# evandez/neuron-descriptions

Hardware: AMD Instinct MI355X
Metric: neuron-descriptions/sec (whole node), 4096 neurons x k=15 exemplars (higher is better)
Workload: dtype f32-equivalent: operands split into (hi,lo) f16 pairs (22 significant bits), 3 f16 MFMAs per product, f32 accumulate

## Files before the change

### neuron-descriptions_amd/csrc/chain.hip

```cpp
#include "common.h"

#include <cstdlib>

namespace milan {

typedef float f32x16 __attribute__((ext_vector_type(16)));
typedef float f32x4 __attribute__((ext_vector_type(4)));
typedef _Float16 f16x8 __attribute__((ext_vector_type(8)));

#define GLOBAL_AS __attribute__((address_space(1)))
#define LDS_AS __attribute__((address_space(3)))

namespace {

__device__ inline f16x8 h8(f32x4 v) { return __builtin_bit_cast(f16x8, v); }

__device__ inline void chain_split8(const float* v, f32x4* hi_out, f32x4* lo_out) {
  split8_rne(v, hi_out, lo_out);
}
__device__ inline void chain_join8(f32x4 hi, f32x4 lo, float* v) { join8_exact(hi, lo, v); }

constexpr int kSRow = 68;
constexpr int kTileFloats = 64 * 64;
constexpr int kConvMaxW = 56;
// ... 5 lines not shown
}

}

template <int P, int NW, bool RES_LDS, int KD, bool XACC, bool PROF = false, int NR = P,
          bool CONV = false, bool C1 = false>
__global__ __launch_bounds__(NW * 64, NW / 4) void chain_kernel(ChainArgs g) {
  long long tprof[8] = {0, 0, 0, 0, 0, 0, 0, 0};
  long long tlast = 0;
  auto stamp = [&](int k) {
    if constexpr (PROF) {
      const long long t = __builtin_readcyclecounter();
      tprof[k] += t - tlast;
      tlast = t;
    }
  };
  if constexpr (PROF) tlast = __builtin_readcyclecounter();
  constexpr int N3 = 4 * P, N1 = NR;
  constexpr int K3 = P + KD;
  constexpr int KS3 = K3 / 16;
  constexpr int NSLAB = N3 / 64;
  constexpr int T3 = K3 / 64;
  constexpr bool RES = KD == 0;
  static_assert(!(RES_LDS && !RES) && K3 % 64 == 0, "chain: configuration");
  constexpr int T1 = N1 / 64;
  constexpr int L = T3 + T1;
  constexpr int NT1 = N1 / 32;
  constexpr int STAGES = RES_LDS ? 7 : 4, AHEAD = STAGES - 1;
  constexpr int INFL = AHEAD - 2;
  constexpr int PIECES = 16 / NW;
  constexpr int C_OPS = RES_LDS ? 8 : (RES ? 10 : 2);
  static_assert(P % 64 == 0 && (NW == 4 || NW == 8), "chain: configuration");
  static_assert(!CONV || (P == 64 && NW == 8 && !RES_LDS), "chain: the conv front needs planes 64");
  static_assert(!C1 || CONV, "chain: c1 in front needs the conv front");
  constexpr int Q1 = C1 ? 1 : 0;
  constexpr int QC = CONV ? 9 + Q1 : 0;
  extern __shared__ __attribute__((aligned(16))) float smem[];

  const int tid = threadIdx.x;
  const int lane = tid & 63;
  const int wave = __builtin_amdgcn_readfirstlane(tid >> 6);
  const int px = lane & 31, half = lane >> 5;
  float sat = 0.f;
  float* ring = smem;
  float* strip = smem + STAGES * kTileFloats + wave * (32 * kSRow);
  float* rstrip = strip;
  float* biasl = smem + STAGES * kTileFloats + NW * (32 * kSRow);

  g.M = live_rows(g.m_live, g.m_live_mul, g.M);
  if ((long)blockIdx.x * (NW * 32) >= g.M) return;
  const long m0 = (long)blockIdx.x * (NW * 32) + wave * 32;
  const long mfrag = (m0 + px < g.M) ? m0 + px : (long)g.M - 1;
  const bool tail = (long)(blockIdx.x + 1) * (NW * 32) > g.M;

  const int lrow = lane >> 4;
  const int lpos = lane & 15;
  auto issue_tile = [&](int q) {
    constexpr int NTILES = QC + NSLAB * L;
    q = q < NTILES ? q : NTILES - 1;
    const float* base;
    long ld;
    if (C1 && q == 0) {
      base = g.W0; ld = 64;
    } else if (CONV && q < QC) {
      base = g.W2 + 64 * (q - Q1); ld = 9 * 64;
    } else {
      const int qc = q - QC;
      const int j = qc / L, qq = qc - j * L;
      if (qq < T3) { base = g.W3 + (long)(64 * j) * K3 + 64 * qq; ld = K3; }
      else { base = g.W1 + (long)(64 * (qq - T3)) * N3 + 64 * j; ld = N3; }
    }
    float* slot = ring + (q % STAGES) * kTileFloats;
#pragma unroll
    for (int i = 0; i < PIECES; ++i) {
      const int pc = wave * PIECES + i;
      const int rr = 4 * pc + lrow;
      const int c = lpos ^ (rr & 15);
      __builtin_amdgcn_global_load_lds(
          (const GLOBAL_AS void*)(base + (long)rr * ld + c * 4),
          (LDS_AS void*)(slot + pc * 256), 16, 0, 0);
    }
  };

  f32x4 t2h[KS3], t2l[KS3];
  float* const cin = smem + STAGES * kTileFloats;
  float* const czero = cin + kConvSlots * 64;
  f32x4 bias2v[CONV ? 8 : 1], bias0v[C1 ? 8 : 1];
  if constexpr (C1) {
#pragma unroll
    for (int s4 = 0; s4 < 4; ++s4) {
      bias0v[2 * s4] = *reinterpret_cast<const f32x4*>(g.bias0 + 16 * s4 + 8 * half);
      bias0v[2 * s4 + 1] = *reinterpret_cast<const f32x4*>(g.bias0 + 16 * s4 + 8 * half + 4);
    }
  }
  if constexpr (CONV) {
    const long wg0 = (long)blockIdx.x * (NW * 32);
    const int nslots = NW * 32 + 2 * (g.cw + 1);
    const int npieces = (nslots + 3) >> 2;
    for (int pc = wave; pc < npieces; pc += NW) {
      const int sl = 4 * pc + lrow;
      long m = wg0 - (g.cw + 1) + sl;
      m = m < 0 ? 0 : (m < g.M ? m : (long)g.M - 1);
      const int c = lpos ^ (sl & 15);
      __builtin_amdgcn_global_load_lds((const GLOBAL_AS void*)(g.C2in + m * 64 + c * 4),
                                       (LDS_AS void*)(cin + pc * 256), 16, 0, 0);
    }
// ... 314 lines not shown
        }

      }
      stamp(2);
      if (qq == T3 - 1) {
        const int n = 64 * j + ecol;
        f32x4 bias0, bias1, rh4[4], rl4[4];
        if constexpr (RES_LDS) {
          wait_vmcnt<(L * PIECES < 63 ? L * PIECES : 63)>();
          bias0 = *reinterpret_cast<const f32x4*>(biasl + n);
          bias1 = *reinterpret_cast<const f32x4*>(biasl + n + 4);
#pragma unroll
          for (int it = 0; it < 4; ++it) {
            const int row = it * 8 + erow;
            const float* rp = rstrip + row * 64;
            const int rsw = row & 1;
            rh4[it] = *reinterpret_cast<const f32x4*>(rp + (((ecol >> 2)) ^ rsw) * 4);
            rl4[it] = *reinterpret_cast<const f32x4*>(rp + (((ecol >> 2) + 1) ^ rsw) * 4);
          }
        } else {
          bias0 = bias3v[0]; bias1 = bias3v[1];
        }
#pragma unroll
        for (int t = 0; t < 2; ++t) {
          acc3[t] = acc3[t] * g.scale3;
          to_strip(acc3[t], t);
        }
#pragma unroll
        for (int it = 0; it < 4; ++it) {
          const int row = it * 8 + erow;
          const long m = m0 + row;
          float* sp = strip + row * kSRow + ecol;
          const f32x4 v0 = *reinterpret_cast<const f32x4*>(sp);
          const f32x4 v1 = *reinterpret_cast<const f32x4*>(sp + 4);
          f32x4 rh, rl;
          if constexpr (RES_LDS) {
            rh = rh4[it]; rl = rl4[it];
          } else if constexpr (RES) {
            rh = res[it][0]; rl = res[it][1];
          }
          float v[8], a[8];
#pragma unroll
          for (int e = 0; e < 4; ++e) {
            v[e] = v0[e] + bias0[e];
            v[4 + e] = v1[e] + bias1[e];
          }
          if constexpr (RES) {
            chain_join8(rh, rl, a);
#pragma unroll
            for (int e = 0; e < 8; ++e) v[e] = v[e] + a[e];
          }
          f32x4 hi, lo;
          split8_relu_rne(v, &hi, &lo, &sat);
          if (m < g.M) {
            float* xp = g.X + m * N3 + n;
            *reinterpret_cast<f32x4*>(xp) = hi;
            *reinterpret_cast<f32x4*>(xp + 4) = lo;
          }
          *reinterpret_cast<f32x4*>(sp) = hi;
          *reinterpret_cast<f32x4*>(sp + 4) = lo;
        }
        if constexpr (!RES_LDS) load_res(j + 1 < NSLAB ? j + 1 : j);
#pragma unroll
        for (int s = 0; s < 4; ++s) {
          const float* fp = strip + px * kSRow + (2 * s + half) * 8;
          xh[s] = *reinterpret_cast<const f32x4*>(fp);
          xl[s] = *reinterpret_cast<const f32x4*>(fp + 4);
        }
        if constexpr (RES_LDS) {
          asm volatile("s_waitcnt lgkmcnt(0)"
                       : "+v"(xh[0]), "+v"(xh[1]), "+v"(xh[2]), "+v"(xh[3]),
                         "+v"(xl[0]), "+v"(xl[1]), "+v"(xl[2]), "+v"(xl[3])
                       :: "memory");
          load_res(j + 1 < NSLAB ? j + 1 : j);
        }
      }
      stamp(3);
      {
        constexpr auto has_c = [](int i) { return ((i % L) + L) % L == T3 - 1; };
        int c_later = 0, c_first = 0;
#pragma unroll
        for (int d = 0; d <= INFL; ++d) {
          c_later += has_c(qq - d) ? 1 : 0;
          c_first += (qq - d >= 0 && has_c(qq - d)) ? 1 : 0;
        }
        const int cnt = (j == 0) ? c_first : c_later;
        constexpr int B = INFL * PIECES;
        if (tail) {
          wait_vmcnt<0>();
        } else {
          switch (cnt) {
            case 0: wait_vmcnt<B>(); break;
            case 1: wait_vmcnt<(B + C_OPS < 63 ? B + C_OPS : 63)>(); break;
            case 2: wait_vmcnt<(B + 2 * C_OPS < 63 ? B + 2 * C_OPS : 63)>(); break;
            default: wait_vmcnt<(B + 3 * C_OPS < 63 ? B + 3 * C_OPS : 63)>(); break;
          }
        }
      }
      stamp(4);
      __builtin_amdgcn_s_barrier();
      stamp(5);
    }
  }
  wait_vmcnt<0>();
  __builtin_amdgcn_s_barrier();

#pragma unroll
// ... 43 lines not shown
}

bool chain_conv_c1_supported(int P, int KD, int NR, int h, int w) {
  return chain_conv_supported(P, KD, NR, h, w) && KD == 64 && NR == 64;
}

bool chain_supported(int P, int KD, int NR) {
  if (NR == 2 * P) return KD == 0 && P == 64;
  if (NR != P) return false;
  if (KD == 0) return P == 64 || P == 128 || P == 256;
  return P == 64 && KD == 64;
}

template <int P, int NW, bool RES_LDS, int KD, bool XACC, bool PROF = false, int NR = P,
          bool CONV = false, bool C1 = false>
static int launch_chain_cfg(const ChainArgs& a, hipStream_t s) {
  size_t lds = sizeof(float) * (size_t)((RES_LDS ? 7 : 4) * kTileFloats +
                                        NW * 32 * kSRow + (RES_LDS ? 4 * P : 0));
  if (CONV) {
    const size_t with_region = sizeof(float) * (size_t)(4 * kTileFloats + kConvSlots * 64 + 64);
    lds = lds > with_region ? lds : with_region;
  }
  auto kern = chain_kernel<P, NW, RES_LDS, KD, XACC, PROF, NR, CONV, C1>;
  MILAN_TRY(ensure_lds_attr(reinterpret_cast<const void*>(kern), (int)lds));
  const int rows = NW * 32;
  const int grid = (a.M + rows - 1) / rows;
  hipLaunchKernelGGL(kern, dim3(grid), dim3(NW * 64), lds, s, a);
  MILAN_CHECK_HIP(hipGetLastError());
  return 0;
}

int launch_chain3(const ChainArgs& a, hipStream_t s);

int launch_chain(const ChainArgs& a0, hipStream_t s) {
  ChainArgs a = a0;
  if (a.status == nullptr) a.status = status_word();
  const int NR = a.NR ? a.NR : a.P;
  MILAN_REQUIRE(chain_supported(a.P, a.KD, NR) && a.M > 0, MILAN_ERR_SHAPE,
                "chain: unsupported planes %d (+%d) -> %d", a.P, a.KD, NR);
  auto al = [](const void* p) { return (reinterpret_cast<uintptr_t>(p) & 15) == 0; };
  const bool conv = a.C2in != nullptr;
  MILAN_REQUIRE(!conv || (chain_conv_supported(a.P, a.KD, NR, a.ch, a.cw) && a.W2 && a.bias2 &&
                          al(a.C2in) && al(a.W2) && al(a.bias2) && a.C2in != a.T1 &&
                          a.M % (a.ch * a.cw) == 0),
                MILAN_ERR_SHAPE, "chain: unsupported 3x3 front (%d x %d images)", a.ch, a.cw);
  const bool c1 = conv && a.W0 != nullptr;
  MILAN_REQUIRE(!c1 || (chain_conv_c1_supported(a.P, a.KD, NR, a.ch, a.cw) && a.bias0 && al(a.W0) &&
                        al(a.bias0)),
                MILAN_ERR_SHAPE, "chain: unsupported c1 front");
  MILAN_REQUIRE((conv || al(a.T2)) && al(a.W3) && al(a.bias3) && al(a.X) && al(a.W1) &&
                    al(a.bias1) && al(a.T1) &&
                    (a.KD ? (a.A2 && al(a.A2) && !a.R) : (a.R && al(a.R))),
                MILAN_ERR_SHAPE, "chain: operands must be 16-byte aligned");
  const double M = a.M, P = a.P, K3 = a.P + a.KD, R1 = NR;
  void* rec = gemm_profile_begin(
      2.0 * M * (4 * P) * (K3 + R1) + (conv ? 2.0 * M * 64 * 576 : 0.0) + (c1 ? 2.0 * M * 64 * 64 : 0.0),
      4.0 * (M * K3 + M * 4 * P * (a.KD ? 1 : 2) + M * R1 + 4 * P * (K3 + R1) +
             (conv ? 64.0 * 576 : 0.0)), s);
  profile_tag_kernel(a.P == 256 ? MILAN_KERNEL_CHAIN_WIDE
                                : (conv ? MILAN_KERNEL_BNECK : MILAN_KERNEL_CHAIN));
  int r;
#if MILAN_EXPERIMENTS
  if (conv && a.KD == 0 && NR == 64 && a.prof)
    r = launch_chain_cfg<64, 8, false, 0, true, true, 64, true>(a, s);
  else
#endif
  if (conv && NR == 128) r = launch_chain_cfg<64, 8, false, 0, false, false, 128, true>(a, s);
  else if (conv && a.KD == 0) r = launch_chain_cfg<64, 8, false, 0, true, false, 64, true>(a, s);
  else if (c1) r = launch_chain_cfg<64, 8, false, 64, true, false, 64, true, true>(a, s);
  else if (conv) r = launch_chain_cfg<64, 8, false, 64, true, false, 64, true>(a, s);
  else if (a.P == 256) r = launch_chain3(a, s);
  else if (a.P == 128) r = launch_chain_cfg<128, 8, false, 0, false>(a, s);
  else if (NR == 128) r = launch_chain_cfg<64, 8, false, 0, false, false, 128>(a, s);
  else if (a.KD == 0) r = launch_chain_cfg<64, 8, false, 0, true>(a, s);
  else r = launch_chain_cfg<64, 8, false, 64, true>(a, s);
  gemm_profile_end(rec, s);
  return r;
}

}
```

### neuron-descriptions_amd/csrc/common.h

```cpp
#pragma once
#include <hip/hip_runtime.h>
#include <stdint.h>
#include <stddef.h>
#include <string>
#include <vector>
#include <map>

#include "../../include/milan_hip.h"

#ifndef MILAN_EXPERIMENTS
#define MILAN_EXPERIMENTS 0
#endif

namespace milan {

void set_error(const char* fmt, ...);
#define MILAN_CHECK_HIP(expr)                                              \
  do {                                                                     \
    hipError_t _e = (expr);                                                \
    if (_e != hipSuccess) {                                                \
      milan::set_error("%s:%d: %s -> %s", __FILE__, __LINE__, #expr,       \
                       hipGetErrorString(_e));                             \
      return (int)_e;                                                      \
    }                                                                      \
// ... 55 lines not shown
  float* Cs;
  unsigned* status;
  int f16;
  const float* Wt;
  int tap_inner;
  const long long* lse_tgt;
  long lse_tgt_stride;
  float* lse_x;
  const int* m_live;
  int m_live_mul;
};

enum OutMode : int { OUT_SCALAR = 0, OUT_VEC4 = 1, OUT_SPLIT8 = 2, OUT_F16 = 3 };

int launch_gemm(const GemmArgs& g, hipStream_t s);
void set_status_word(unsigned* word);
unsigned* status_word();
void profile_tag_kernel(int family);
int launch_zero_fill(void* p, size_t bytes, hipStream_t s);
int launch_f32_to_split(const float* src, long ld_src, float* dst, long ld_dst,
                        long rows, int K, float scale, hipStream_t s);
int gemm_profile_enable(int enable);
int ensure_lds_attr(const void* kern, int bytes);
int device_cus8(int* out);
void* gemm_profile_begin(double flops, double bytes, hipStream_t s);
void gemm_profile_end(void* rec, hipStream_t s);

struct ChainArgs {
  const float* T2;
  const float* W3;
  const float* bias3;
  const float* R;
  float* X;
  const float* W1;
  const float* bias1;
  float* T1;
  int M, P;
  const float* A2;
  int KD;
  float scale3, scale1;
  long long* prof;
  int NR;
  unsigned* status;
  const int* m_live;
  int m_live_mul;
  const float* C2in;
  const float* W2;
  const float* bias2;
  float scale2;
  int ch, cw;
  const float* W0;
  const float* bias0;
  float scale0;
};
bool chain_supported(int P, int KD, int NR = 0);
bool chain_conv_supported(int P, int KD, int NR, int h, int w);
bool chain_conv_c1_supported(int P, int KD, int NR, int h, int w);
int launch_chain(const ChainArgs& a, hipStream_t s);
struct StemArgs {
  const float* in;
  const float* ws;
  const float* bias;
  float acc_scale;
  const float* scale;
  const float* shift;
  float* raw;
  float* y;
  const int* bbox;
  const float* zero;
  int n, H, G, h1, w1, hp, wp;
  int tiles_y, tiles_x;
  int debug;
  unsigned* status;
  const unsigned char* in_u8;
  const unsigned* lut;
  const int* order;
  int W;
  const int* n_live;
};
bool stem_fused_supported(int cout, int Kp);
int launch_stem_fused(const StemArgs& a, hipStream_t s);
struct Conv3Args {
  const float* in;
  const float* ws;
  const float* bias;
  float acc_scale;
  float* out;
  const float* zero;
  int n, h, w;
  int tiles_y, tiles_x;
  int debug;
  long long* prof;
  unsigned* status;
  const int* n_live;
};
bool conv3_p64_supported(int cin, int cout, int kh, int kw, int stride, int pad);
int launch_conv3_p64(const Conv3Args& a, hipStream_t s);
bool gemm_profile_active();
int gemm_profile_read(double* ms, double* flops, long long* launches);
int profile_read_stages(double* table );
int profile_read_kernels(double* table );
class StageScope {
 public:
  StageScope(int stage, hipStream_t s);
  ~StageScope();
  StageScope(const StageScope&) = delete;
// ... 252 lines not shown
```

### neuron-descriptions_amd/csrc/decoder.hip

```cpp
#include "common.h"
#include <limits>
#include <optional>

namespace milan {

static constexpr float kFloatMin = -3.402823466e+38f;

static const Tensor* find(milan_ctx* c, const std::string& name) {
  auto it = c->raw.find(name);
  return it == c->raw.end() ? nullptr : &it->second;
}

__global__ void pack_rows_kernel(const float* __restrict__ src, int n, int k,
                                 int kp, float* __restrict__ dst) {
  const long total = (long)n * kp;
  for (long idx = blockIdx.x * (long)blockDim.x + threadIdx.x; idx < total;
       idx += (long)gridDim.x * blockDim.x) {
    const int r = idx / kp, col = idx - (long)r * kp;
    dst[idx] = col < k ? src[(long)r * k + col] : 0.f;
  }
}

__device__ inline int lstm_source_row(int i, int hidden) {
  if (!hidden) return i;
// ... 1655 lines not shown
    int in_dim = El;
    for (int l = 0; l < d.lm_layers; ++l) {
      float* h_next = hs + ((size_t)(cur ^ 1) * d.lm_layers + l) * layer_sz;
      float* hn = nx.h + (long)l * nx.rows * Hl;
      float* cn = nx.c + (long)l * nx.rows * Hl;
      const LinearW& w = c->lm_cat[l];
      GemmArgs g = linear_args(in, in_dim, w.ws, w.b, hn, Hl, R, w.n, w.k, EPI_LSTM, c->zero,
                               q.gc + l * layer_sz, Hl);
      g.C2 = cn; g.Cs = h_next;
      g.a_split = 1;
      g.acc_scale = w.ws_inv;
      g.Cin = in_dim;
      g.A2 = q.gh + l * layer_sz; g.K1 = in_dim; g.H2 = 1; g.W2d = 1; g.stride2 = 1;
      g.a2_pix_stride = Hl; g.a2_img_stride = Hl;
      g.m_live = U1; g.m_live_mul = 1;
      MILAN_TRY(launch_gemm(g, s));
      in = h_next;
      in_dim = Hl;
    }
    hipLaunchKernelGGL(lm_gather_rows_kernel, dim3(nblk((long)R * (Hl / 4), 8192)), dim3(256), 0, s,
                       (const float4*)in, q.par + (size_t)p2 * R, U2, Hl / 4, (float4*)q.gv);
    hipLaunchKernelGGL(lm_gather_tok_kernel, dim3(nblk(R)), dim3(256), 0, s, seqs, (long)L, t + 1,
                       q.urow + (size_t)p2 * R, U2, q.tgt_c);
    {
      GemmArgs g = linear_args(q.gv, Hl, c->lm_out.ws, c->lm_out.b, b->lm_logits, V, R,
                               c->lm_out.n, c->lm_out.k, EPI_BIAS, c->zero);
      g.a_split = 1;
      g.acc_scale = c->lm_out.ws_inv;
      g.epilogue = EPI_LSE;
      g.ldc = 2 * nb;
      g.lse_tgt = reinterpret_cast<const long long*>(q.tgt_c);
      g.lse_tgt_stride = 1;
      g.lse_x = b->lm_logits + (size_t)R * 2 * nb;
      g.m_live = U2; g.m_live_mul = 1;
      MILAN_TRY(launch_gemm(g, s));
    }
    hipLaunchKernelGGL(lm_accumulate_lse_kernel, dim3((R + 3) / 4), dim3(256), 0, s,
                       b->lm_logits, nb, b->lm_logits + (size_t)R * 2 * nb, R, seqs, (long)L, t,
                       seq_len, len_div, d.stop_index, b->lm_alive, total,
                       q.cls + (size_t)p2 * R);
    cur ^= 1;
  }
  MILAN_CHECK_HIP(hipGetLastError());
  return 0;
}

static int lm_score_impl(milan_ctx* c, const int64_t* seqs, int rows, int L,
                         const int32_t* seq_len, int len_div, float* total,
                         DecBuf* b, hipStream_t s, int group = 1,
                         float* dedup_scratch = nullptr, size_t dedup_floats = 0) {
  const milan_dims& d = c->d;
  MILAN_REQUIRE(d.has_lm && c->lm_out.w, MILAN_ERR_NO_LM,
                "cannot use MI/rerank decoding without an LM");
  const size_t st_bytes =
      sizeof(float) * (size_t)b->lm[0].rows * d.lm_hidden_size * d.lm_layers;
  MILAN_TRY(launch_zero_fill(b->lm[0].h, st_bytes, s));
  MILAN_TRY(launch_zero_fill(b->lm[0].c, st_bytes, s));
  if (L < 2) {
    MILAN_TRY(launch_zero_fill(total, sizeof(float) * rows, s));
    return 0;
  }
  int cur = 0;
  const bool split = lm_split_ok(c, rows) && (long)rows == b->lm[0].rows;
  static const bool lse_on = !(getenv("MILAN_LM_LSE") && atoi(getenv("MILAN_LM_LSE")) == 0);
  const bool lse = lse_on && d.vocab_size % 4 == 0 && d.vocab_size >= 256;
  if (split)
    MILAN_TRY(launch_zero_fill(b->lm_gates, sizeof(float) * (size_t)rows * d.lm_hidden_size * d.lm_layers, s));
  static const bool dedup_on = !(getenv("MILAN_LM_DEDUP") && atoi(getenv("MILAN_LM_DEDUP")) == 0);
  if (dedup_on && split && lse && group > 1 && group <= 256 && rows % group == 0 && dedup_scratch &&
      d.lm_hidden_size % 4 == 0 &&
      lm_dedup_floats(d, (size_t)rows, L, rows / group) <= dedup_floats)
    return lm_score_dedup(c, seqs, rows, L, group, seq_len, len_div, total, b, dedup_scratch, s);
  for (int t = 0; t + 1 < L; ++t) {
    hipLaunchKernelGGL(gather_col_kernel, dim3(nblk(rows)), dim3(256), 0, s, seqs,
                       (long)rows, (long)L, t, b->tok);
    if (split && lse) {
      const int nb = (d.vocab_size + 63) / 64;
      MILAN_TRY(lm_step_split(c, b->tok, rows, b->lm[cur], b->lm[cur ^ 1],
                              b->lm_gates, cur, b->lm_logits, s, seqs + t + 1, (long)L));
      hipLaunchKernelGGL(lm_accumulate_lse_kernel, dim3((rows + 3) / 4), dim3(256), 0, s,
                         b->lm_logits, nb, b->lm_logits + (size_t)rows * 2 * nb, rows, seqs,
                         (long)L, t, seq_len, len_div, d.stop_index, b->lm_alive, total);
      cur ^= 1;
      continue;
    }
    if (split)
      MILAN_TRY(lm_step_split(c, b->tok, rows, b->lm[cur], b->lm[cur ^ 1],
                              b->lm_gates, cur, b->lm_logits, s));
    else
      MILAN_TRY(lm_step(c, b->tok, rows, b->lm[cur], b->lm[cur ^ 1], b->lm_emb,
                        b->lm_gates, b->lm_logits, s));
    hipLaunchKernelGGL(lm_accumulate_kernel, dim3(rows), dim3(256), 0, s,
                       b->lm_logits, d.vocab_size, seqs, (long)L, t, seq_len,
                       len_div, d.stop_index, b->lm_alive, total);
    cur ^= 1;
  }
  MILAN_CHECK_HIP(hipGetLastError());
  return 0;
}

int decoder_lm_score(milan_ctx* c, const int64_t* seqs, int rows, int L,
                     const int32_t* seq_len, float* out, Arena& ws,
                     hipStream_t s) {
  MILAN_REQUIRE(c->finalized, MILAN_ERR_STATE, "weights not finalized");
  MILAN_REQUIRE(c->d.has_lm && c->lm_out.w, MILAN_ERR_NO_LM,
                "cannot use MI/rerank decoding without an LM");
  MILAN_REQUIRE(rows > 0 && L >= 1, MILAN_ERR_SHAPE, "lm_score: empty input");
  DecBuf b;
  dec_plan(c, rows, 1, 1, 1, true, ws, &b);
  c->scratch = ws.off <= ws.size ? b.scratch : nullptr;
  c->scratch_floats = b.scratch_floats;
  MILAN_REQUIRE(ws.off <= ws.size, MILAN_ERR_WORKSPACE,
                "lm_score: workspace too small (%zu needed)", ws.off);
  return lm_score_impl(c, seqs, rows, L, seq_len, 1, out, &b, s);
}

int decoder_lm_logprobs(milan_ctx* c, const int64_t* seqs, int rows, int L,
                        float* out, Arena& ws, hipStream_t s) {
  MILAN_REQUIRE(c->finalized, MILAN_ERR_STATE, "weights not finalized");
  MILAN_REQUIRE(c->d.has_lm && c->lm_out.w, MILAN_ERR_NO_LM,
                "cannot use MI/rerank decoding without an LM");
  MILAN_REQUIRE(rows > 0 && L >= 1, MILAN_ERR_SHAPE, "lm_logprobs: empty input");
  const milan_dims& d = c->d;
  DecBuf b;
  dec_plan(c, rows, 1, 1, 1, true, ws, &b);
// ... 174 lines not shown
```

### neuron-descriptions_amd/csrc/encoder.hip

```cpp
#include "common.h"
#include <optional>
#include <vector>

#include <cstdlib>

namespace milan {

static constexpr float kBnEps = 1e-5f;

__global__ void pack_conv_kernel(const float* __restrict__ w, int cout, int cin,
                                 int cinp, int kh, int kw, int kp,
                                 const float* __restrict__ gamma,
                                 const float* __restrict__ beta,
                                 const float* __restrict__ mean,
                                 const float* __restrict__ var,
                                 float* __restrict__ wp,
                                 float* __restrict__ bias) {
  const long total = (long)cout * kp;
  for (long idx = blockIdx.x * (long)blockDim.x + threadIdx.x; idx < total;
       idx += (long)gridDim.x * blockDim.x) {
    const int o = idx / kp, k = idx - (long)o * kp;
    const int tap = k / cinp, i = k - tap * cinp;
    float v = 0.f;
    if (tap < kh * kw && i < cin) {
// ... 852 lines not shown
        for (int dx = -1; dx <= 1; ++dx) {
          const int yy = y + dy, xx = x + dx;
          if (yy >= 0 && yy < h && xx >= 0 && xx < w) v |= s[k - 1][yy * w + xx];
        }
      s[k][p] = v;
    }
    __syncthreads();
  }
  for (int k = 0; k < 3; ++k) {
    int count = 0;
    int* out = loc + ((long)k * n + j) * P;
    for (int p0 = 0; p0 < P; p0 += 64) {
      const int p = p0 + lane;
      const bool nz = p < P && s[k][p];
      const unsigned long long m = __ballot(nz);
      if (nz) out[count + __popcll(m & ((1ull << lane) - 1ull))] = p;
      count += __popcll(m);
    }
    if (lane == 0) cnt[k * n + j] = count;
  }
}

__global__ __launch_bounds__(256) void tail_scan_kernel(const int* __restrict__ cnt, int n,
                                                        int* __restrict__ off, int* __restrict__ U) {
  __shared__ int tmp[256];
  const int k = blockIdx.x, tid = threadIdx.x;
  int base = 0;
  for (int j0 = 0; j0 < n; j0 += 256) {
    const int j = j0 + tid;
    const int v = j < n ? cnt[(long)k * n + j] : 0;
    tmp[tid] = v;
    __syncthreads();
    for (int o = 1; o < 256; o <<= 1) {
      const int add = tid >= o ? tmp[tid - o] : 0;
      __syncthreads();
      tmp[tid] += add;
      __syncthreads();
    }
    if (j < n) off[(long)k * n + j] = base + tmp[tid] - v;
    base += tmp[255];
    __syncthreads();
  }
  if (tid == 0) U[k] = base;
}

__global__ void tail_fill_kernel(const int* __restrict__ loc, const int* __restrict__ cnt,
                                 const int* __restrict__ off, int n, int P, int* __restrict__ rows) {
  const int j = blockIdx.x, k = blockIdx.y;
  const int c = cnt[k * n + j], o = off[k * n + j];
  for (int i = threadIdx.x; i < c; i += blockDim.x)
    rows[(long)k * n * P + o + i] = j * P + loc[((long)k * n + j) * P + i];
}

template <bool SCATTER>
__global__ void tail_rows_kernel(const float4* __restrict__ src, const int* __restrict__ idx,
                                 const int* __restrict__ live, int w4, float4* __restrict__ dst) {
  const long total = (long)*live * w4;
  for (long i = blockIdx.x * (long)blockDim.x + threadIdx.x; i < total;
       i += (long)gridDim.x * blockDim.x) {
    const long u = i / w4;
    const int q = (int)(i - u * w4);
    if (SCATTER) dst[(long)idx[u] * w4 + q] = src[i];
    else dst[i] = src[(long)idx[u] * w4 + q];
  }
}

__global__ void tail_im2col_kernel(const float4* __restrict__ t1, const int* __restrict__ rows,
                                   const int* __restrict__ live, int h, int w, int C,
                                   float4* __restrict__ acol) {
  const int per = 9 * C / 4, P = h * w, c4 = C / 4;
  const long total = (long)*live * per;
  for (long i = blockIdx.x * (long)blockDim.x + threadIdx.x; i < total;
       i += (long)gridDim.x * blockDim.x) {
    const long u = i / per;
    const int q = (int)(i - u * per);
    const int sl = q / 72, r = q - sl * 72, tap = r >> 3, f = r & 7;
    const int row = rows[u];
    const int j = row / P, p = row - j * P;
    const int y = p / w + tap / 3 - 1, x = p % w + tap % 3 - 1;
    float4 v = make_float4(0.f, 0.f, 0.f, 0.f);
    if (y >= 0 && y < h && x >= 0 && x < w)
      v = t1[((long)j * P + y * w + x) * c4 + sl * 8 + f];
    acol[i] = v;
  }
}

struct EncPlan {
  Levels lv;
  int h1, w1, hp, wp;
  float *in4, *raw, *x0, *x1, *ds, *t1, *t2;
  size_t x_sz, t1_sz, t2_sz;
  int *list_idx, *list_n;
  float* list_w;
  int* bbox;
  int* poison;
  int *order, *bbox_c, *count;
  int *tail_loc, *tail_cnt, *tail_off, *tail_rows, *tail_U;
};

static int conv_out(int h, int k, int s, int p) { return (h + 2 * p - k) / s + 1; }

static int plan(const milan_ctx* c, int n, int H, int W, Arena& a, EncPlan* pl) {
  const int wd = c->d.trunk_width;
  pl->h1 = conv_out(H, 7, 2, 3); pl->w1 = conv_out(W, 7, 2, 3);
  pl->hp = conv_out(pl->h1, 3, 2, 1); pl->wp = conv_out(pl->w1, 3, 2, 1);
  Levels& lv = pl->lv;
  lv.h[0] = pl->h1; lv.w[0] = pl->w1;
  lv.h[1] = pl->hp; lv.w[1] = pl->wp;
  for (int l = 2; l < 5; ++l) {
    lv.h[l] = conv_out(lv.h[l - 1], 3, 2, 1);
    lv.w[l] = conv_out(lv.w[l - 1], 3, 2, 1);
  }
  long off = 0;
  for (int l = 0; l < 5; ++l) { lv.off[l] = off; off += (long)lv.h[l] * lv.w[l]; }
  lv.per_image = off;
  const int exp = c->d.trunk_kind == MILAN_TRUNK_BASIC ? 1 : 4;
  size_t x_sz = (size_t)pl->hp * pl->wp * wd, t1_sz = 0, t2_sz = 0;
  for (int li = 0; li < 4; ++li) {
    const size_t planes = (size_t)wd << li;
    const size_t in_px = (size_t)lv.h[li == 0 ? 1 : li] * lv.w[li == 0 ? 1 : li];
    const size_t out_px = (size_t)lv.h[li + 1] * lv.w[li + 1];
    x_sz = x_sz > out_px * planes * exp ? x_sz : out_px * planes * exp;
    t1_sz = t1_sz > in_px * planes ? t1_sz : in_px * planes;
    t2_sz = t2_sz > out_px * planes ? t2_sz : out_px * planes;
  }
  pl->x_sz = x_sz; pl->t1_sz = t1_sz; pl->t2_sz = t2_sz;
  pl->in4 = a.get<float>((size_t)n * H * (W + 2) * 4);
  pl->raw = a.get<float>((size_t)n * pl->h1 * pl->w1 * wd);
  pl->x0 = a.get<float>((size_t)n * x_sz);
  pl->x1 = a.get<float>((size_t)n * x_sz);
  pl->ds = a.get<float>((size_t)n * x_sz);
  pl->t1 = a.get<float>((size_t)n * t1_sz);
  pl->t2 = a.get<float>((size_t)n * t2_sz);
  pl->list_idx = a.get<int>((size_t)n * lv.per_image);
  pl->list_w = a.get<float>((size_t)n * lv.per_image);
  pl->list_n = a.get<int>((size_t)n * 5);
  pl->bbox = a.get<int>((size_t)n * 4);
  pl->poison = a.get<int>((size_t)n);
  pl->order = a.get<int>((size_t)n);
  pl->bbox_c = a.get<int>((size_t)n * 4);
  pl->count = a.get<int>(4);
  {
    const size_t P4 = (size_t)lv.h[4] * lv.w[4];
    pl->tail_loc = a.get<int>(3 * (size_t)n * P4);
    pl->tail_rows = a.get<int>(3 * (size_t)n * P4);
    pl->tail_cnt = a.get<int>(3 * (size_t)n);
    pl->tail_off = a.get<int>(3 * (size_t)n);
    pl->tail_U = a.get<int>(4);
  }
  return 0;
}

static int encoder_sub_batch() {
  static int v = 0;
  if (v == 0) {
    const char* e = getenv("MILAN_ENC_SUB");
    v = e ? atoi(e) : 9600;
    if (v < 1) v = 9600;
  }
  return v;
}

static void alexnet_workspace_dry(const milan_ctx* c, int n, int H, int W,
                                  Arena& a);

size_t encoder_workspace(const milan_ctx* c, int n_images, int H, int W) {
  Arena a; a.dry = true;
  const int sub = encoder_sub_batch();
  const int n = n_images < sub ? n_images : sub;
  if (c->d.trunk_kind == MILAN_TRUNK_NONE) return 0;
  if (c->d.trunk_kind == MILAN_TRUNK_ALEXNET) {
    alexnet_workspace_dry(c, n, H, W, a);
    return a.off;
  }
  EncPlan pl;
  plan(c, n, H, W, a, &pl);
  return a.off;
}

static GemmArgs conv_args(const ConvW& cw, const float* in, int n, int H, int W,
                          float* out, int epi, const float* aux,
                          const float* zero, int* Ho, int* Wo,
                          bool split = false, bool scaled_bias = true) {
  GemmArgs g{};
  *Ho = conv_out(H, cw.kh, cw.stride, cw.pad);
  *Wo = conv_out(W, cw.kw, cw.stride, cw.pad);
  g.A = in; g.W = cw.w; g.bias = cw.bias; g.aux = aux; g.C = out;
  g.M = n * (*Ho) * (*Wo); g.N = cw.cout; g.K = cw.K; g.Kp = cw.Kp;
  g.ldc = cw.cout; g.ldaux = cw.cout;
  g.H = H; g.Wd = W; g.Cin = cw.cin; g.Ho = *Ho; g.Wo = *Wo;
  g.KH = cw.kh; g.KW = cw.kw; g.stride = cw.stride; g.pad = cw.pad;
  g.a_pix_stride = cw.cin;
  g.a_img_stride = (long)H * W * cw.cin;
  g.epilogue = epi; g.zero = zero;
  g.flop_k = cw.kh * cw.kw * cw.cin_real;
  if (split) {
    g.W = cw.ws; g.a_split = 1; g.out_split = 1; g.aux_split = aux != nullptr;
    g.acc_scale = cw.ws_inv;
    g.W3 = cw.ws3;
    g.Wt = cw.wst;
    if (scaled_bias && cw.bias_s) g.bias = cw.bias_s;
  }
// ... 30 lines not shown
  for (int lo = 0; lo < n; lo += sub) {
    const int cnt = n - lo < sub ? n - lo : sub;
    Arena a = ws;
    const char* im = (const char*)images + (size_t)lo * 3 * H * W * isz;
    const char* mk = masks ? (const char*)masks + (size_t)lo * H * W * msz : nullptr;
    MILAN_TRY(encoder_run_batch(c, im, image_dtype, mk, mask_dtype, cnt, H, W,
                                features + (size_t)lo * c->d.feature_size, a, s));
    if (a.off > ws.off) ws.off = a.off > ws.size ? ws.size : ws.off;
  }
  return 0;
}

int encoder_run_spatial(milan_ctx* c, const void* images, int image_dtype,
                        const void* masks, int mask_dtype, int n, int H, int W,
                        float* out, Arena& ws, hipStream_t s) {
  MILAN_REQUIRE(c->d.trunk_kind != MILAN_TRUNK_ALEXNET, MILAN_ERR_ARG,
                "spatial encoding needs a ResNet trunk");
  Arena dry; dry.dry = true;
  EncPlan pl;
  plan(c, 1, H, W, dry, &pl);
  const int C = (c->d.trunk_kind == MILAN_TRUNK_BASIC ? c->d.trunk_width
                                                      : c->d.trunk_width * 4) << 3;
  const size_t per_image = (size_t)pl.lv.h[4] * pl.lv.w[4] * C;
  const int sub = encoder_sub_batch();
  const size_t isz = image_dtype == MILAN_DTYPE_U8 ? 1 : 4;
  const size_t msz = mask_dtype == MILAN_DTYPE_U8 ? 1 : 4;
  for (int lo = 0; lo < n; lo += sub) {
    const int cnt = n - lo < sub ? n - lo : sub;
    Arena a = ws;
    const char* im = (const char*)images + (size_t)lo * 3 * H * W * isz;
    const char* mk = masks ? (const char*)masks + (size_t)lo * H * W * msz : nullptr;
    MILAN_TRY(encoder_run_batch(c, im, image_dtype, mk, mask_dtype, cnt, H, W,
                                nullptr, a, s, out + lo * per_image));
    if (a.off > ws.off) ws.off = a.off > ws.size ? ws.size : ws.off;
  }
  return 0;
}

static int encoder_run_batch(milan_ctx* c, const void* images, int image_dtype,
                             const void* masks, int mask_dtype, int n, int H,
                             int W, float* features, Arena& ws, hipStream_t s,
                             float* spatial_out) {
  const bool spatial = spatial_out != nullptr;
  MILAN_REQUIRE(!spatial || c->d.trunk_kind != MILAN_TRUNK_ALEXNET, MILAN_ERR_ARG,
                "spatial encoding needs a ResNet trunk");
  MILAN_REQUIRE(c->stem.w != nullptr, MILAN_ERR_STATE,
                "encoder weights were not uploaded");
  MILAN_REQUIRE(n > 0 && H >= 1 && W >= 1, MILAN_ERR_SHAPE,
                "encode: need n>0 and H,W>=1 (got n=%d H=%d W=%d)", n, H, W);
  if (c->d.trunk_kind == MILAN_TRUNK_ALEXNET)
    return alexnet_run_batch(c, images, image_dtype, masks, mask_dtype, n, H, W,
                             features, ws, s);
  EncPlan pl;
  plan(c, n, H, W, ws, &pl);
  MILAN_REQUIRE(ws.off <= ws.size, MILAN_ERR_WORKSPACE,
                "encode: workspace too small (%zu needed, %zu given)", ws.off,
                ws.size);
  const int wd = c->d.trunk_width;
  const int F = c->d.feature_size;
  int* const poison = image_dtype == MILAN_DTYPE_F32 ? pl.poison : nullptr;
  auto track = [&](const float* t, long count) -> int {
    if (c->calib == nullptr || count <= 0) return 0;
    const int blocks = (int)((count + 255) / 256 < 4096 ? (count + 255) / 256 : 4096);
    hipLaunchKernelGGL(act_absmax_kernel, dim3(blocks), dim3(256), 0, s, t, count, c->calib);
    MILAN_CHECK_HIP(hipGetLastError());
    return 0;
  };

  std::optional<StageScope> stage;
  stage.emplace(MILAN_STAGE_ENC_INPUT, s);
  if (spatial) {
  } else if (masks == nullptr || mask_dtype == MILAN_DTYPE_U8)
    hipLaunchKernelGGL(mask_pyramid_kernel<uint8_t>, dim3(n, 5), dim3(256), 0, s,
                       (const uint8_t*)masks, H, W, pl.lv, pl.list_idx,
                       pl.list_w, pl.list_n, pl.bbox);
  else
    hipLaunchKernelGGL(mask_pyramid_kernel<float>, dim3(n, 5), dim3(256), 0, s,
                       (const float*)masks, H, W, pl.lv, pl.list_idx, pl.list_w,
                       pl.list_n, pl.bbox);
  MILAN_CHECK_HIP(hipGetLastError());

  const int n_all = n;
  const int* order = nullptr;
  const int* live = nullptr;
  if (!spatial && masks != nullptr && image_dtype == MILAN_DTYPE_U8 && c->calib == nullptr &&
      (c->fusion & MILAN_FUSE_SKIP_EMPTY)) {
    hipLaunchKernelGGL(compact_images_kernel, dim3(1), dim3(1024), 0, s, pl.list_n, n_all,
                       pl.bbox, pl.order, pl.bbox_c, pl.count);
    MILAN_CHECK_HIP(hipGetLastError());
    MILAN_TRY(launch_zero_fill(features, sizeof(float) * (size_t)n_all * c->d.feature_size, s));
    order = pl.order;
    live = pl.count;
  }
  const int* const bbox = order ? pl.bbox_c : pl.bbox;
  auto launch_live = [&](GemmArgs g) -> int {
    g.m_live = live;
    g.m_live_mul = g.Ho * g.Wo;
    return launch_gemm(g, s);
  };

  bool split = c->precision == MILAN_PRECISION_SPLIT_F16 && wd % 8 == 0;
  for (int li = 0; li < 4 && split; ++li)
    for (const Bottleneck& b : c->blocks[li])
      split = split && b.c1.ws && b.c2.ws && (b.basic || b.c3.ws) &&
              (!b.has_down || b.down.ws);
  bool fast = split && c->trunk_f16 && !spatial && c->d.trunk_kind == MILAN_TRUNK_BOTTLENECK;
  for (int li = 2; li < 4 && fast; ++li)
    for (const Bottleneck& b : c->blocks[li])
      fast = fast && !b.basic && b.c1.wf && b.c2.wf && (b.has_down ? b.c3d.wf != nullptr : b.c3.wf != nullptr);
  const bool pair_stem = split && c->stem_pair.ws != nullptr;
  const int G = (W + 2) / 2;

// ... 110 lines not shown
        StageScope scope(MILAN_STAGE_ENC_STEM, s);
        MILAN_TRY(launch_stem_fused(sa, s));
      }
      MILAN_TRY(pool(pl.raw, 0, wd, 0));
    } else {
    {
      StageScope scope(MILAN_STAGE_ENC_STEM, s);
      MILAN_TRY(launch_live(g));
    }
    MILAN_TRY(pool(pl.raw, 0, wd, 0));
    stage.emplace(MILAN_STAGE_ENC_STEM_TAIL, s);
    const long total = (long)n * pl.hp * pl.wp * (wd / (split ? 8 : 4));
    const int blocks = (int)((total + 255) / 256 < 16384 ? (total + 255) / 256 : 16384);
    if (split)
      hipLaunchKernelGGL(bn_relu_maxpool_split_kernel, dim3(blocks), dim3(256), 0,
                         s, pl.raw, n, pl.h1, pl.w1, wd, pl.hp, pl.wp,
                         c->bn1_scale_s, c->bn1_shift_s, pl.x0, c->status, live);
    else
      hipLaunchKernelGGL(bn_relu_maxpool_kernel, dim3(blocks), dim3(256), 0, s,
                         (const float4*)pl.raw, n, pl.h1, pl.w1, wd / 4, pl.hp,
                         pl.wp, (const float4*)c->bn1_scale,
                         (const float4*)c->bn1_shift, (float4*)pl.x0, live);
    MILAN_CHECK_HIP(hipGetLastError());
    stage.reset();
    }
    if (c->calib && !split) {
      MILAN_TRY(track(pl.x0, (long)n * pl.hp * pl.wp * wd));
    }
  }

  auto gemm_t = [&](const GemmArgs& g) -> int {
    MILAN_TRY(launch_live(g));
    if (c->calib && !split) MILAN_TRY(track(g.C, (long)g.M * g.N));
    return 0;
  };
  const int P4 = pl.lv.h[4] * pl.lv.w[4];
  bool tail = split && !fast && !spatial && masks != nullptr && c->calib == nullptr &&
              (c->fusion & MILAN_FUSE_SPARSE_TAIL) && c->d.trunk_kind == MILAN_TRUNK_BOTTLENECK &&
              c->blocks[3].size() >= 2 && P4 >= 1 && P4 <= kTailMaxP;
  if (tail) {
    const Bottleneck& lb = c->blocks[3].back();
    const size_t need = (size_t)P4 * ((size_t)2 * lb.c1.cin + lb.c3.cout + (size_t)11 * lb.c1.cout);
    tail = need <= (size_t)pl.h1 * pl.w1 * wd;
  }
  if (tail) {
    hipLaunchKernelGGL(tail_sets_kernel, dim3(n), dim3(64), 0, s, pl.list_idx, pl.list_n, pl.lv,
                       order, live, n, pl.tail_loc, pl.tail_cnt);
    hipLaunchKernelGGL(tail_scan_kernel, dim3(3), dim3(256), 0, s, pl.tail_cnt, n, pl.tail_off,
                       pl.tail_U);
    hipLaunchKernelGGL(tail_fill_kernel, dim3(n, 3), dim3(64), 0, s, pl.tail_loc, pl.tail_cnt,
                       pl.tail_off, n, P4, pl.tail_rows);
    MILAN_CHECK_HIP(hipGetLastError());
  }
  auto tail_block_ok = [&](const Bottleneck& b) {
    return !b.basic && !b.has_down && b.c1.ws && b.c2.ws && b.c2.wst && b.c3.ws && b.c1.bias_s &&
           b.c2.bias_s && b.c3.bias_s && b.c1.kh == 1 && b.c1.kw == 1 && b.c1.stride == 1 &&
           b.c2.kh == 3 && b.c2.kw == 3 && b.c2.stride == 1 && b.c2.pad == 1 && b.c3.kh == 1 &&
           b.c3.kw == 1 && b.c3.stride == 1 && b.c1.K == b.c1.Kp && b.c2.K == b.c2.Kp &&
           b.c3.K == b.c3.Kp && b.c1.cout % 32 == 0 && b.c2.cin == b.c1.cout &&
           b.c2.cout == b.c1.cout && b.c3.cin == b.c1.cout && b.c3.cout == b.c1.cin &&
           b.c1.cin % 4 == 0;
  };
  auto tail_block = [&](const Bottleneck& b, const float* X, float* Y, float* T1, int hh,
                        int ww, int kM, int kO) -> int {
    const long rows_all = (long)n * P4;
    const int Cin = b.c1.cin, P = b.c1.cout, Cout = b.c3.cout;
    float* xg = pl.raw;
    float* t1c = xg + rows_all * Cin;
    float* acol = t1c + rows_all * P;
    float* t2c = acol + rows_all * 9 * P;
    float* rg = t2c + rows_all * P;
    float* yc = rg + rows_all * Cin;
    const int* rowsM = pl.tail_rows + (long)kM * n * P4;
    const int* rowsO = pl.tail_rows + (long)kO * n * P4;
    const int* UM = pl.tail_U + kM;
    const int* UO = pl.tail_U + kO;
    auto blocks_for = [](long items) { return (int)((items + 255) / 256 < 8192 ? (items + 255) / 256 : 8192); };
    auto lin = [&](const float* A, int K, const ConvW& cw, const float* W, float* C, int N, int epi,
                   const float* aux, const int* U) -> int {
      GemmArgs g = linear_args(A, K, W, cw.bias_s, C, N, (int)rows_all, N, K, epi, c->zero, aux, N);
      g.a_split = 1; g.out_split = 1; g.aux_split = aux != nullptr;
      g.acc_scale = cw.ws_inv;
      g.flop_k = cw.kh * cw.kw * cw.cin_real;
      g.m_live = U; g.m_live_mul = 1;
      return launch_gemm(g, s);
    };
    hipLaunchKernelGGL(tail_rows_kernel<false>, dim3(blocks_for(rows_all * (Cin / 4))), dim3(256), 0, s,
                       (const float4*)X, rowsM, UM, Cin / 4, (float4*)xg);
    MILAN_TRY(lin(xg, Cin, b.c1, b.c1.ws, t1c, P, EPI_BIAS_RELU, nullptr, UM));
    hipLaunchKernelGGL(tail_rows_kernel<true>, dim3(blocks_for(rows_all * (P / 4))), dim3(256), 0, s,
                       (const float4*)t1c, rowsM, UM, P / 4, (float4*)T1);
    hipLaunchKernelGGL(tail_im2col_kernel, dim3(blocks_for(rows_all * (9 * P / 4))), dim3(256), 0, s,
                       (const float4*)T1, rowsO, UO, hh, ww, P, (float4*)acol);
    MILAN_TRY(lin(acol, 9 * P, b.c2, b.c2.wst, t2c, P, EPI_BIAS_RELU, nullptr, UO));
    hipLaunchKernelGGL(tail_rows_kernel<false>, dim3(blocks_for(rows_all * (Cin / 4))), dim3(256), 0, s,
                       (const float4*)X, rowsO, UO, Cin / 4, (float4*)rg);
    MILAN_TRY(lin(t2c, P, b.c3, b.c3.ws, yc, Cout, EPI_BIAS_RES_RELU, rg, UO));
    hipLaunchKernelGGL(tail_rows_kernel<true>, dim3(blocks_for(rows_all * (Cout / 4))), dim3(256), 0, s,
                       (const float4*)yc, rowsO, UO, Cout / 4, (float4*)Y);
    MILAN_CHECK_HIP(hipGetLastError());
    return 0;
  };

  float *x = pl.x0, *y = pl.x1;
  int h = pl.hp, w = pl.wp, col = wd;
  bool t1_ready = false;
// ... 98 lines not shown
                            nb.c1.K == nb.c1.Kp && b.c3.bias && nb.c1.bias;
        h2 = conv_out(h1, b.c2.kh, b.c2.stride, b.c2.pad);
        w2 = conv_out(w1, b.c2.kw, b.c2.stride, b.c2.pad);
        chain_plain = shapes && !b.has_down && chain_supported(chain_P, 0, chain_NR);
        chain_ds = shapes && b.has_down && b.c3d.ws && b.down.kh == 1 &&
                   b.down.kw == 1 && b.down.stride == 1 && h2 == h &&
                   w2 == w && chain_supported(chain_P, b.down.cin, chain_NR);
      }
      const bool conv_front =
          (chain_plain || chain_ds) && (c->fusion & MILAN_FUSE_BNECK) && b.c2.K == b.c2.Kp &&
          b.c2.bias_s && conv3_p64_supported(b.c2.cin, b.c2.cout, b.c2.kh, b.c2.kw, b.c2.stride,
                                             b.c2.pad) &&
          chain_conv_supported(chain_P, chain_ds ? b.down.cin : 0, chain_NR, h1, w1);
      const bool c1_front =
          conv_front && c1_pending && chain_ds && b.c1.ws && b.c1.bias_s && b.c1.kh == 1 &&
          b.c1.kw == 1 && b.c1.stride == 1 && b.c1.cin == 64 && b.c1.cout == 64 &&
          b.c1.K == b.c1.Kp && h1 == h && w1 == w &&
          chain_conv_c1_supported(chain_P, b.down.cin, chain_NR, h1, w1);
      if (c1_pending && !c1_front) MILAN_TRY(gemm_t(g1));
      if (conv_front) {
      } else if (split && (c->fusion & MILAN_FUSE_CONV3) && b.c2.K == b.c2.Kp &&
          conv3_p64_supported(b.c2.cin, b.c2.cout, b.c2.kh, b.c2.kw, b.c2.stride,
                              b.c2.pad)) {
        Conv3Args ca{};
        ca.in = t1buf; ca.ws = b.c2.ws; ca.bias = b.c2.bias_s; ca.acc_scale = b.c2.ws_inv;
        ca.out = pl.t2; ca.zero = c->zero; ca.n = n; ca.h = h1; ca.w = w1;
        ca.n_live = live;
        MILAN_TRY(launch_conv3_p64(ca, s));
      } else {
        MILAN_TRY(gemm_t(g2));
      }
      const float* identity = x;
      if (chain_plain || chain_ds) {
        const Bottleneck& nb = *nbp;
        ChainArgs ca{};
        ca.T2 = pl.t2; ca.X = y; ca.W1 = nb.c1.ws; ca.bias1 = nb.c1.bias_s;
        ca.T1 = t1buf; ca.M = n * h2 * w2; ca.P = chain_P; ca.scale1 = nb.c1.ws_inv;
        ca.NR = chain_NR;
        ca.m_live = live; ca.m_live_mul = h2 * w2;
        if (conv_front) {
          ca.C2in = t1buf; ca.W2 = b.c2.ws; ca.bias2 = b.c2.bias_s; ca.scale2 = b.c2.ws_inv;
          ca.ch = h1; ca.cw = w1;
          ca.T2 = nullptr; ca.T1 = t1alt;
          if (c1_front) {
            ca.C2in = x; ca.W0 = b.c1.ws; ca.bias0 = b.c1.bias_s; ca.scale0 = b.c1.ws_inv;
          }
        }
        if (chain_plain) {
          ca.W3 = b.c3.ws; ca.bias3 = b.c3.bias_s; ca.R = x; ca.scale3 = b.c3.ws_inv;
        } else {
          ca.W3 = b.c3d.ws; ca.bias3 = b.c3d.bias_s; ca.A2 = x; ca.KD = b.down.cin;
          ca.scale3 = b.c3d.ws_inv;
        }
        MILAN_TRY(launch_chain(ca, s));
        if (conv_front) { float* tt = t1buf; t1buf = t1alt; t1alt = tt; }
        t1_ready = true;
        float* tmp = x; x = y; y = tmp;
        h = h2; w = w2;
        continue;
      }
      if (b.has_down && split && b.c3d.ws && b.c3d.cout > 64) {
        int h3, w3;
        GemmArgs g3 = conv_args(b.c3d, pl.t2, n, h2, w2, y, EPI_BIAS_RELU,
                                nullptr, c->zero, &h3, &w3, true);
        g3.Cin = b.c3.cin;
        g3.a_pix_stride = b.c3.cin;
        g3.a_img_stride = (long)h2 * w2 * b.c3.cin;
        g3.A2 = x; g3.K1 = b.c3.K; g3.H2 = h; g3.W2d = w;
        g3.stride2 = b.down.stride;
        g3.a2_pix_stride = b.down.cin;
        g3.a2_img_stride = (long)h * w * b.down.cin;
        g3.flop_k = b.c3.K + b.down.K;
        MILAN_TRY(gemm_t(g3));
        float* tmp = x; x = y; y = tmp;
        h = h3; w = w3;
        continue;
      }
      if (b.has_down) {
        int hd, wdn;
        GemmArgs gd = conv_args(b.down, x, n, h, w, pl.ds, EPI_BIAS, nullptr,
                                c->zero, &hd, &wdn, split);
        MILAN_TRY(gemm_t(gd));
        identity = pl.ds;
      }
      GemmArgs g3 = conv_args(b.c3, pl.t2, n, h2, w2, y, EPI_BIAS_RES_RELU,
                              identity, c->zero, &h3, &w3, split);
      MILAN_TRY(gemm_t(g3));
      float* tmp = x; x = y; y = tmp;
      h = h3; w = w3;
    }
    stage.reset();
    const int C = (c->d.trunk_kind == MILAN_TRUNK_BASIC ? wd : wd * 4) << li;
    MILAN_REQUIRE(h == pl.lv.h[li + 1] && w == pl.lv.w[li + 1], MILAN_ERR_SHAPE,
                  "internal: stage %d geometry mismatch", li + 1);
    MILAN_TRY(pool(x, li + 1, C, col));
    col += C;
  }
  if (spatial) {
    const int C = (c->d.trunk_kind == MILAN_TRUNK_BASIC ? wd : wd * 4) << 3;
    const long rows = (long)n * h * w;
    if (split) {
      const long total = rows * (C / 8);
      const int blocks = (int)((total + 255) / 256 < 16384 ? (total + 255) / 256 : 16384);
      hipLaunchKernelGGL(split_to_f32_kernel, dim3(blocks), dim3(256), 0, s, x,
                         total, spatial_out, 1.f / c->act_scale);
      MILAN_CHECK_HIP(hipGetLastError());
// ... 253 lines not shown
```

Before: 1351.

## Skip chain output stores for pixels not consumed downstream at stage boundary

Adds a per-pixel keep bitmask, built by a new kernel from the strided downsample grid and the mask-selected feature list, so the stage-boundary chain kernel only writes the X rows that later layers actually read. This cuts global store traffic in the last bottleneck of a stage. The LM scoring path also moves its state zero-fills below the dedup early return so that path no longer pays for them. A poison-workspace debug option is included to catch reads of rows that were skipped. The cost is an extra zero-fill plus the mask-building launch, and any consumer that reads a skipped row will silently get stale data.

```diff
diff --git a/neuron-descriptions_amd/csrc/chain.hip b/neuron-descriptions_amd/csrc/chain.hip
--- a/neuron-descriptions_amd/csrc/chain.hip
+++ b/neuron-descriptions_amd/csrc/chain.hip
@@ -81,6 +81,13 @@
   const long m0 = (long)blockIdx.x * (NW * 32) + wave * 32;
   const long mfrag = (m0 + px < g.M) ? m0 + px : (long)g.M - 1;
   const bool tail = (long)(blockIdx.x + 1) * (NW * 32) > g.M;
+  constexpr bool XKEEP = CONV && NR == 2 * P;
+  unsigned keepw = 0xffffffffu;
+  if constexpr (XKEEP) {
+    typedef const unsigned __attribute__((address_space(4)))* KWord;
+    if (g.xkeep != nullptr)
+      keepw = ((KWord)(uintptr_t)g.xkeep)[((long)blockIdx.x * (NW * 32) + wave * 32) >> 5];
+  }
 
   const int lrow = lane >> 4;
   const int lpos = lane & 15;
@@ -501,7 +508,9 @@
           }
           f32x4 hi, lo;
           split8_relu_rne(v, &hi, &lo, &sat);
-          if (m < g.M) {
+          bool st = m < g.M;
+          if constexpr (XKEEP) st = st && ((keepw >> row) & 1u);
+          if (st) {
             float* xp = g.X + m * N3 + n;
             *reinterpret_cast<f32x4*>(xp) = hi;
             *reinterpret_cast<f32x4*>(xp + 4) = lo;
@@ -651,6 +660,8 @@
                     al(a.bias1) && al(a.T1) &&
                     (a.KD ? (a.A2 && al(a.A2) && !a.R) : (a.R && al(a.R))),
                 MILAN_ERR_SHAPE, "chain: operands must be 16-byte aligned");
+  MILAN_REQUIRE(a.xkeep == nullptr || (conv && NR == 2 * a.P), MILAN_ERR_ARG,
+                "chain: a store set needs the stage-boundary launch with the conv front");
   const double M = a.M, P = a.P, K3 = a.P + a.KD, R1 = NR;
   void* rec = gemm_profile_begin(
       2.0 * M * (4 * P) * (K3 + R1) + (conv ? 2.0 * M * 64 * 576 : 0.0) + (c1 ? 2.0 * M * 64 * 64 : 0.0),
diff --git a/neuron-descriptions_amd/csrc/common.h b/neuron-descriptions_amd/csrc/common.h
--- a/neuron-descriptions_amd/csrc/common.h
+++ b/neuron-descriptions_amd/csrc/common.h
@@ -131,6 +131,7 @@
   const float* W0;
   const float* bias0;
   float scale0;
+  const unsigned* xkeep;
 };
 bool chain_supported(int P, int KD, int NR = 0);
 bool chain_conv_supported(int P, int KD, int NR, int h, int w);
diff --git a/neuron-descriptions_amd/csrc/decoder.hip b/neuron-descriptions_amd/csrc/decoder.hip
--- a/neuron-descriptions_amd/csrc/decoder.hip
+++ b/neuron-descriptions_amd/csrc/decoder.hip
@@ -1731,10 +1731,6 @@
   const milan_dims& d = c->d;
   MILAN_REQUIRE(d.has_lm && c->lm_out.w, MILAN_ERR_NO_LM,
                 "cannot use MI/rerank decoding without an LM");
-  const size_t st_bytes =
-      sizeof(float) * (size_t)b->lm[0].rows * d.lm_hidden_size * d.lm_layers;
-  MILAN_TRY(launch_zero_fill(b->lm[0].h, st_bytes, s));
-  MILAN_TRY(launch_zero_fill(b->lm[0].c, st_bytes, s));
   if (L < 2) {
     MILAN_TRY(launch_zero_fill(total, sizeof(float) * rows, s));
     return 0;
@@ -1743,13 +1739,17 @@
   const bool split = lm_split_ok(c, rows) && (long)rows == b->lm[0].rows;
   static const bool lse_on = !(getenv("MILAN_LM_LSE") && atoi(getenv("MILAN_LM_LSE")) == 0);
   const bool lse = lse_on && d.vocab_size % 4 == 0 && d.vocab_size >= 256;
-  if (split)
-    MILAN_TRY(launch_zero_fill(b->lm_gates, sizeof(float) * (size_t)rows * d.lm_hidden_size * d.lm_layers, s));
   static const bool dedup_on = !(getenv("MILAN_LM_DEDUP") && atoi(getenv("MILAN_LM_DEDUP")) == 0);
   if (dedup_on && split && lse && group > 1 && group <= 256 && rows % group == 0 && dedup_scratch &&
       d.lm_hidden_size % 4 == 0 &&
       lm_dedup_floats(d, (size_t)rows, L, rows / group) <= dedup_floats)
     return lm_score_dedup(c, seqs, rows, L, group, seq_len, len_div, total, b, dedup_scratch, s);
+  const size_t st_bytes =
+      sizeof(float) * (size_t)b->lm[0].rows * d.lm_hidden_size * d.lm_layers;
+  MILAN_TRY(launch_zero_fill(b->lm[0].h, st_bytes, s));
+  MILAN_TRY(launch_zero_fill(b->lm[0].c, st_bytes, s));
+  if (split)
+    MILAN_TRY(launch_zero_fill(b->lm_gates, sizeof(float) * (size_t)rows * d.lm_hidden_size * d.lm_layers, s));
   for (int t = 0; t + 1 < L; ++t) {
     hipLaunchKernelGGL(gather_col_kernel, dim3(nblk(rows)), dim3(256), 0, s, seqs,
                        (long)rows, (long)L, t, b->tok);
diff --git a/neuron-descriptions_amd/csrc/encoder.hip b/neuron-descriptions_amd/csrc/encoder.hip
--- a/neuron-descriptions_amd/csrc/encoder.hip
+++ b/neuron-descriptions_amd/csrc/encoder.hip
@@ -928,6 +928,44 @@
     rows[(long)k * n * P + o + i] = j * P + loc[((long)k * n + j) * P + i];
 }
 
+constexpr int kStoreSetMaxP = 4096;
+
+__global__ __launch_bounds__(256) void store_set_kernel(
+    const int* __restrict__ list_idx, const int* __restrict__ list_n, Levels lv, int level,
+    int stride, const int* __restrict__ order, const int* __restrict__ live,
+    unsigned* __restrict__ keep) {
+  __shared__ unsigned char s[kStoreSetMaxP];
+  const int j = blockIdx.x, lane = threadIdx.x & 63;
+  if (live != nullptr && j >= *live) return;
+  const int img = order ? order[j] : j;
+  const int w = lv.w[level], P = lv.h[level] * w;
+  for (int p = threadIdx.x; p < P; p += 256) {
+    const int y = p / w, x = p - y * w;
+    s[p] = (y % stride == 0 && x % stride == 0) ? 1 : 0;
+  }
+  __syncthreads();
+  const long base = (long)img * lv.per_image + lv.off[level];
+  const int c = list_n[img * 5 + level];
+  for (int i = threadIdx.x; i < c; i += 256) s[list_idx[base + i]] = 1;
+  __syncthreads();
+  for (int p0 = 0; p0 < P; p0 += 256) {
+    const int p = p0 + threadIdx.x;
+    const unsigned long long b = __ballot(p < P && s[p]);
+    const long m = (long)j * P + p;
+    const int o = (int)(m & 31);
+    if (lane == 0 || o == 0) {
+      const unsigned bits = (unsigned)((b >> lane) << o);
+      if (bits) atomicOr(keep + (m >> 5), bits);
+    }
+  }
+}
+
+__global__ void poison_workspace_kernel(float4* __restrict__ p, long n4) {
+  for (long i = blockIdx.x * (long)blockDim.x + threadIdx.x; i < n4;
+       i += (long)gridDim.x * blockDim.x)
+    p[i] = make_float4(1e30f, 1e30f, 1e30f, 1e30f);
+}
+
 template <bool SCATTER>
 __global__ void tail_rows_kernel(const float4* __restrict__ src, const int* __restrict__ idx,
                                  const int* __restrict__ live, int w4, float4* __restrict__ dst) {
@@ -972,6 +1010,8 @@
   int* poison;
   int *order, *bbox_c, *count;
   int *tail_loc, *tail_cnt, *tail_off, *tail_rows, *tail_U;
+  unsigned* keep1;
+  size_t keep1_words;
 };
 
 static int conv_out(int h, int k, int s, int p) { return (h + 2 * p - k) / s + 1; }
@@ -1024,6 +1064,8 @@
     pl->tail_off = a.get<int>(3 * (size_t)n);
     pl->tail_U = a.get<int>(4);
   }
+  pl->keep1_words = ((size_t)n * lv.h[1] * lv.w[1] + 255) / 256 * 8;
+  pl->keep1 = a.get<unsigned>(pl->keep1_words);
   return 0;
 }
 
@@ -1160,12 +1202,22 @@
     return alexnet_run_batch(c, images, image_dtype, masks, mask_dtype, n, H, W,
                              features, ws, s);
   EncPlan pl;
+  const size_t ws_begin = ws.off;
   plan(c, n, H, W, ws, &pl);
   MILAN_REQUIRE(ws.off <= ws.size, MILAN_ERR_WORKSPACE,
                 "encode: workspace too small (%zu needed, %zu given)", ws.off,
                 ws.size);
   const int wd = c->d.trunk_width;
   const int F = c->d.feature_size;
+  {
+    const char* const pe = getenv("MILAN_POISON_WORKSPACE");
+    const bool poison_ws = pe && atoi(pe);
+    if (poison_ws && ws.base != nullptr) {
+      hipLaunchKernelGGL(poison_workspace_kernel, dim3(8192), dim3(256), 0, s,
+                         (float4*)(ws.base + ws_begin), (long)((ws.off - ws_begin) / 16));
+      MILAN_CHECK_HIP(hipGetLastError());
+    }
+  }
   int* const poison = image_dtype == MILAN_DTYPE_F32 ? pl.poison : nullptr;
   auto track = [&](const float* t, long count) -> int {
     if (c->calib == nullptr || count <= 0) return 0;
@@ -1382,6 +1434,10 @@
                        pl.tail_off, n, P4, pl.tail_rows);
     MILAN_CHECK_HIP(hipGetLastError());
   }
+  const char* const chain_env = getenv("MILAN_CHAIN");
+  const bool store_sets = split && !fast && !spatial && masks != nullptr && c->calib == nullptr &&
+                          c->d.trunk_kind == MILAN_TRUNK_BOTTLENECK &&
+                          !(chain_env && *chain_env && !(atoi(chain_env) & 128));
   auto tail_block_ok = [&](const Bottleneck& b) {
     return !b.basic && !b.has_down && b.c1.ws && b.c2.ws && b.c2.wst && b.c3.ws && b.c1.bias_s &&
            b.c2.bias_s && b.c3.bias_s && b.c1.kh == 1 && b.c1.kw == 1 && b.c1.stride == 1 &&
@@ -1586,6 +1642,16 @@
           ca.W3 = b.c3d.ws; ca.bias3 = b.c3d.bias_s; ca.A2 = x; ca.KD = b.down.cin;
           ca.scale3 = b.c3d.ws_inv;
         }
+        if (store_sets && li == 0 && last_of_stage && conv_front && chain_plain &&
+            chain_NR == 2 * chain_P && nb.has_down && nb.down.kh == 1 && nb.down.kw == 1 &&
+            nb.down.pad == 0 && nb.down.stride >= 1 && nb.down.cin == b.c3.cout &&
+            h2 == pl.lv.h[1] && w2 == pl.lv.w[1] && h2 * w2 <= kStoreSetMaxP) {
+          MILAN_TRY(launch_zero_fill(pl.keep1, sizeof(unsigned) * pl.keep1_words, s));
+          hipLaunchKernelGGL(store_set_kernel, dim3(n), dim3(256), 0, s, pl.list_idx, pl.list_n,
+                             pl.lv, 1, nb.down.stride, order, live, pl.keep1);
+          MILAN_CHECK_HIP(hipGetLastError());
+          ca.xkeep = pl.keep1;
+        }
         MILAN_TRY(launch_chain(ca, s));
         if (conv_front) { float* tt = t1buf; t1buf = t1alt; t1alt = tt; }
         t1_ready = true;
```

Result: no change. 1356, median of 6 (+0.4%).
